# MMintLab/gelslim_depth

Hardware: AMD Instinct MI355X
Metric: train frames/sec (320x427) at batch 32 (higher is better)
Workload: dtype f32

## Files before the change

### gelslim_depth_amd/csrc/gsd_convT_wgrad.hip

```cpp
#include "gsd_wgrad_host.h"

template <int WM, int WN>
__global__ __launch_bounds__(256) void convT_wgrad_kernel(const WgradParams P) {
  constexpr int MT = 4, NTB = 4;
  constexpr int BMw = WM * 64, BNw = WN * 64;
  constexpr int DS = 66;

  extern __shared__ __attribute__((aligned(16))) float smem[];
  float* Al = smem;
  float* Xl = smem + BMw * DS;

  const int tid = threadIdx.x, lane = tid & 63, wave = tid >> 6;
  const int wm = wave / WN, wn = wave % WN;
  const int j = lane >> 4, l16 = lane & 15;

  const int per_split = P.mblocks * P.nblocks;
  const int split = blockIdx.x / per_split;
  const int rem = blockIdx.x - split * per_split;
  const int mb = rem % P.mblocks, nb = rem / P.mblocks;
  const int m0 = mb * BMw, n0 = nb * BNw;
  const int s_begin = (int)((long long)split * P.stages_total / P.splits);
  const int s_end = (int)((long long)(split + 1) * P.stages_total / P.splits);
  const int HW = P.H * P.W;

  f32x4 acc[MT][NTB];
#pragma unroll
  for (int m = 0; m < MT; ++m)
#pragma unroll
    for (int t = 0; t < NTB; ++t) acc[m][t] = f32x4{0.f, 0.f, 0.f, 0.f};

  const int q = tid & 63;
  const int lrow = tid >> 6;

  for (int stage = s_begin; stage < s_end; ++stage) {
    const int n = stage / P.tiles_flat;
    const int p = (stage - n * P.tiles_flat) * 64 + q;
    const bool pix_ok = p < HW;
    const int h = pix_ok ? p / P.W : 0;
    const int w = pix_ok ? p - h * P.W : 0;
    __syncthreads();
#pragma unroll
    for (int i = 0; i < BMw / 8; ++i) {
      const int rr = lrow + 4 * i;
      const int co = (m0 >> 2) + (rr >> 1);
      const int kh = rr & 1;
      float2 v = make_float2(0.f, 0.f);
      if (pix_ok && co < P.dy.C)
        v = *reinterpret_cast<const float2*>(P.dy.p + (long long)n * P.dy.ns + (long long)co * P.dy.cs +
                                             (long long)(2 * h + kh) * P.dy.W + 2 * w);
      const int mrow = (rr >> 1) * 4 + kh * 2;
      Al[mrow * DS + q] = v.x;
      Al[(mrow + 1) * DS + q] = v.y;
    }
#pragma unroll
    for (int i = 0; i < BNw / 4; ++i) {
      const int ch = lrow + 4 * i;
      const int c = n0 + ch;
      float v = 0.f;
      if (pix_ok && c < P.a0.C) {
        v = P.a0.p[(long long)n * P.a0.ns + (long long)c * P.a0.cs + p];
        if (P.a0.scale != nullptr) v = apply_affine(v, P.a0.scale[c], P.a0.shift[c], P.a0.relu);
        else if (P.a0.relu) v = fmaxf(v, 0.f);
      }
      Xl[ch * DS + q] = v;
    }
    __syncthreads();
    const int a_base = (wm * 64 + l16) * DS + j;
    const int b_base = (wn * 64 + l16) * DS + j;
    for (int s = 0; s < 16; ++s) {
      float a[MT], b[NTB];
#pragma unroll
      for (int m = 0; m < MT; ++m) a[m] = Al[a_base + m * 16 * DS + 4 * s];
#pragma unroll
      for (int t = 0; t < NTB; ++t) b[t] = Xl[b_base + t * 16 * DS + 4 * s];
#pragma unroll
      for (int m = 0; m < MT; ++m)
#pragma unroll
        for (int t = 0; t < NTB; ++t) acc[m][t] = mfma16(a[m], b[t], acc[m][t]);
    }
  }

#pragma unroll
  for (int m = 0; m < MT; ++m)
#pragma unroll
    for (int reg = 0; reg < 4; ++reg) {
      const int mr = m0 + wm * 64 + m * 16 + j * 4 + reg;
      if (mr < P.M) {
#pragma unroll
        for (int t = 0; t < NTB; ++t) {
          const int col = n0 + wn * 64 + t * 16 + l16;
          if (col < P.Ncols) P.slabs[((size_t)split * P.M + mr) * P.Ncols + col] = acc[m][t][reg];
        }
      }
    }
}

__device__ __attribute__((aligned(16))) const float gsd_zero16_wg[4] = {0.f, 0.f, 0.f, 0.f};
typedef float f32x2 __attribute__((ext_vector_type(2)));
template <int XM>
__global__ __launch_bounds__(256, 2) void convT_wgrad_dma_kernel(const WgradParams P) {
  constexpr bool BX = XM >= 1, AX = XM == 2;
  constexpr int MT = 4, NTB = 4, BMw = 128, BNw = 128, DS = 66, DSB = BX ? 64 : DS;
  extern __shared__ __attribute__((aligned(16))) float smem[];
  float* Al = smem;
  float* Bl = smem + BMw * DS;
  const int tid = threadIdx.x, lane = tid & 63;
  const int wave = __builtin_amdgcn_readfirstlane(tid >> 6);
  const int wm = wave >> 1, wn = wave & 1;
  const int j = lane >> 4, l16 = lane & 15;

  const int lid = xcd_swizzle(blockIdx.x, gridDim.x);
  const int per_split = P.mblocks * P.nblocks;
  const int split = lid / per_split;
  const int rem = lid - split * per_split;
  const int mb = rem % P.mblocks, nb = rem / P.mblocks;
  const int m0 = mb * BMw, n0 = nb * BNw;
  const int s_begin = (int)((long long)split * P.stages_total / P.splits);
  const int s_end = (int)((long long)(split + 1) * P.stages_total / P.splits);
  const int HW = P.H * P.W;

  float sc[NTB], sh[NTB], lo[NTB];
#pragma unroll
  for (int t = 0; t < NTB; ++t) {
    const int c = n0 + wn * 64 + t * 16 + l16;
    sc[t] = 1.f; sh[t] = 0.f; lo[t] = -__builtin_inff();
    if (c < P.a0.C) {
      if (P.a0.scale != nullptr) { sc[t] = P.a0.scale[c]; sh[t] = P.a0.shift[c]; }
      if (P.a0.relu) lo[t] = 0.f;
    }
  }

  f32x4 acc[MT][NTB];
#pragma unroll
  for (int m = 0; m < MT; ++m)
#pragma unroll
    for (int t = 0; t < NTB; ++t) acc[m][t] = f32x4{0.f, 0.f, 0.f, 0.f};

  const int a_off = AX ? (wm * 32 + (l16 >> 1)) * 128 + 2 * (j & 1) + (l16 & 1) : (wm * 64 + l16) * DS + j;
  const int a_lr = lane >> 5, a_q = lane & 31;
  const int a_sp = a_q ^ ((2 * wave + a_lr) & 7);
  const int b_off = (wn * 64 + l16) * DSB + j;
  const int b_lr = lane >> 4;
  const int b_piece = (lane & 15) ^ ((4 * wave + b_lr) & 15);
  for (int stage = s_begin; stage < s_end; ++stage) {
    const int n = stage / P.tiles_flat;
    const int p = (stage - n * P.tiles_flat) * 64 + lane;
    const bool pix_ok = p < HW;
    const int h = pix_ok ? p / P.W : 0;
    const int w = pix_ok ? p - h * P.W : 0;
    __syncthreads();
    f32x2 a_fix[AX ? BMw / 16 : 1];
    bool a_str = false;
    if constexpr (AX) {
      const int pa = (stage - n * P.tiles_flat) * 64 + 2 * a_sp;
      const bool pa_ok = pa < HW;
      const int ha = pa_ok ? pa / P.W : 0, wa = pa_ok ? pa - ha * P.W : 0;
      a_str = pa_ok && wa == P.W - 1;
      const bool pb_ok = pa + 1 < HW;
      const float* abase = P.dy.p + (long long)n * P.dy.ns + (long long)(2 * ha) * P.dy.W + 2 * wa;
#pragma unroll
      for (int i = 0; i < BMw / 16; ++i) {
        const int R = 2 * (wave + 4 * i) + a_lr;
        const int m = m0 + 2 * R;
        const float* src = abase + (long long)(m >> 2) * P.dy.cs + ((m >> 1) & 1) * P.dy.W;
        const float* gsrc = (pa_ok && m < P.M) ? src : &gsd_zero16_wg[0];
        float* dstp = Al + (wave + 4 * i) * 256;
        __builtin_amdgcn_global_load_lds(gsrc, dstp, 16, 0, 0);
        a_fix[i] = f32x2{0.f, 0.f};
        if (a_str && pb_ok && m < P.M) a_fix[i] = *reinterpret_cast<const f32x2*>(src + 2 * P.dy.W - 2 * wa);
      }
    } else {
      const float* abase = P.dy.p + (long long)n * P.dy.ns + (long long)(2 * h) * P.dy.W + 2 * w;
#pragma unroll 4
      for (int i = 0; i < BMw / 4; ++i) {
        const int row = wave + 4 * i;
        const int m = m0 + row;
        const float* gsrc = (pix_ok && m < P.M) ? abase + (long long)(m >> 2) * P.dy.cs + ((m >> 1) & 1) * P.dy.W + (m & 1) : &gsd_zero16_wg[0];
        __builtin_amdgcn_global_load_lds(gsrc, Al + row * DS, 4, 0, 0);
      }
    }
    if constexpr (BX) {
      const int p0 = (stage - n * P.tiles_flat) * 64 + 4 * b_piece;
      const bool pc_ok = p0 < HW;
      const float* bbase = P.a0.p + (long long)n * P.a0.ns + p0;
#pragma unroll 4
      for (int i = 0; i < BNw / 16; ++i) {
        const int ch = 4 * (wave + 4 * i) + b_lr;
        const int c = n0 + ch;
        const float* gsrc = (pc_ok && c < P.a0.C) ? bbase + (long long)c * P.a0.cs : &gsd_zero16_wg[0];
        float* dstp = Bl + (wave + 4 * i) * (4 * DSB);
        __builtin_amdgcn_global_load_lds(gsrc, dstp, 16, 0, 0);
      }
    } else {
      const float* bbase = P.a0.p + (long long)n * P.a0.ns + p;
#pragma unroll 4
      for (int i = 0; i < BNw / 4; ++i) {
        const int ch = wave + 4 * i;
        const int c = n0 + ch;
        const float* gsrc = (pix_ok && c < P.a0.C) ? bbase + (long long)c * P.a0.cs : &gsd_zero16_wg[0];
        __builtin_amdgcn_global_load_lds(gsrc, Bl + ch * DS, 4, 0, 0);
      }
    }
    if constexpr (AX) {
      __builtin_amdgcn_s_waitcnt(0x0F70);
      if (a_str) {
#pragma unroll
        for (int i = 0; i < BMw / 16; ++i)
          *reinterpret_cast<f32x2*>(&Al[(wave + 4 * i) * 256 + lane * 4 + 2]) = a_fix[i];
      }
      __syncthreads();
    } else {
      gsd_dma_barrier();
    }
    float an[MT], bn[NTB];
#pragma unroll
    for (int m = 0; m < MT; ++m) an[m] = AX ? Al[a_off + m * 8 * 128 + 4 * ((j >> 1) ^ (l16 >> 1))] : Al[a_off + m * 16 * DS];
#pragma unroll
    for (int t = 0; t < NTB; ++t) bn[t] = Bl[b_off + t * 16 * DSB + (BX ? 4 * l16 : 0)];
    for (int s = 0; s < 16; ++s) {
      float a[MT], b[NTB];
#pragma unroll
      for (int m = 0; m < MT; ++m) a[m] = an[m];
#pragma unroll
      for (int t = 0; t < NTB; ++t) b[t] = fmaxf(fmaf(bn[t], sc[t], sh[t]), lo[t]);
      const int sn = s + 1 < 16 ? s + 1 : s;
#pragma unroll
      for (int m = 0; m < MT; ++m)
        an[m] = AX ? Al[a_off + m * 8 * 128 + 4 * ((2 * sn + (j >> 1)) ^ (l16 >> 1))] : Al[a_off + m * 16 * DS + 4 * sn];
#pragma unroll
      for (int t = 0; t < NTB; ++t) bn[t] = Bl[b_off + t * 16 * DSB + 4 * (BX ? (sn ^ l16) : sn)];
#pragma unroll
      for (int m = 0; m < MT; ++m)
#pragma unroll
        for (int t = 0; t < NTB; ++t) acc[m][t] = mfma16(a[m], b[t], acc[m][t]);
    }
  }
#pragma unroll
  for (int m = 0; m < MT; ++m)
#pragma unroll
    for (int reg = 0; reg < 4; ++reg) {
      const int mr = m0 + wm * 64 + m * 16 + j * 4 + reg;
      if (mr < P.M) {
#pragma unroll
        for (int t = 0; t < NTB; ++t) {
          const int col = n0 + wn * 64 + t * 16 + l16;
          if (col < P.Ncols) P.slabs[((size_t)split * P.M + mr) * P.Ncols + col] = acc[m][t][reg];
        }
      }
    }
}

template <int LANES>
__global__ __launch_bounds__(LANES == 1 ? 256 : 64 * LANES) void convT_wgrad_reduce_kernel(const float* __restrict__ slabs,
                                                                                           float* __restrict__ dw, int splits, int M,
                                                                                           int Ncols) {
  constexpr int EL = LANES == 1 ? 256 : 64;
  const long long per = (long long)M * Ncols;
  const int el = threadIdx.x % EL, sl = threadIdx.x / EL;
  __shared__ float red[LANES][EL];
  for (long long e0 = (long long)blockIdx.x * EL; e0 < per; e0 += (long long)gridDim.x * EL) {
    const long long e = e0 + el;
    const bool ok = e < per;
    float s = 0.f;
    if (ok)
      for (int k = sl; k < splits; k += LANES) s += slabs[(size_t)k * per + e];
    if (LANES > 1) {
      red[sl][el] = s;
      __syncthreads();
      if (sl == 0) {
        s = 0.f;
#pragma unroll
        for (int i = 0; i < LANES; ++i) s += red[i][el];
      }
    }
    if (sl == 0 && ok) dw[(size_t)(e % Ncols) * M + (size_t)(e / Ncols)] = s;
    if (LANES > 1) __syncthreads();
  }
}

__global__ void sum_planes_stage1(const float* __restrict__ x, int N, int K, long long HW, float* __restrict__ ws) {
  const int k = blockIdx.x, g = blockIdx.y, G = gridDim.y;
  const long long total = (long long)N * HW;
  const long long per = (total + G - 1) / G;
  const long long b = (long long)g * per, e = b + per < total ? b + per : total;
  double s = 0.0;
  long long i = b + threadIdx.x;
  long long n = i / HW, p = i - n * HW;
  const long long step = blockDim.x, nstep = step / HW, pstep = step - nstep * HW;
  for (; i < e; i += step) {
    s += (double)x[((size_t)n * K + k) * HW + p];
    n += nstep;
    p += pstep;
    if (p >= HW) {
      p -= HW;
      ++n;
    }
  }
  __shared__ double red[16];
  s = wave_sum_d(s);
  if ((threadIdx.x & 63) == 0) red[threadIdx.x >> 6] = s;
  __syncthreads();
  if (threadIdx.x == 0) {
    double t = 0.0;
    for (int i = 0; i < (int)(blockDim.x >> 6); ++i) t += red[i];
    ws[(size_t)k * G + g] = (float)t;
  }
}
__global__ void sum_planes_stage2(const float* __restrict__ ws, int K, int G, float* __restrict__ out) {
  const int k = blockIdx.x * blockDim.x + threadIdx.x;
  if (k < K) {
    double s = 0.0;
    for (int g = 0; g < G; ++g) s += (double)ws[(size_t)k * G + g];
    out[k] = (float)s;
  }
}

namespace {

struct ConvTWgPlan {
  bool wide;
  int mblocks, nblocks, tiles_flat, stages_total, splits;
  int64_t slab_elems;
};

ConvTWgPlan plan_convT_wgrad(int N, int H, int W, int M, int Ncols) {
  ConvTWgPlan p;
  p.wide = M <= 64;
  p.mblocks = ceil_div(M, p.wide ? 64 : 128);
  p.nblocks = ceil_div(Ncols, p.wide ? 256 : 128);
  p.tiles_flat = ceil_div(H * W, 64);
  p.stages_total = N * p.tiles_flat;
  p.splits = wgrad_pick_splits(gsd_env_int("GSD_WGRAD_BLOCKS", 512), p.mblocks * p.nblocks, p.stages_total);
  p.slab_elems = (int64_t)p.splits * M * Ncols;
  return p;
}

void launch_convT_wgrad_reduce(const float* slabs, float* dw, int splits, int M, int Ncols, hipStream_t st) {
  const int lanes = splits >= 64 ? 16 : splits >= 8 ? 4 : 1;
  const int64_t blocks = ceil_div64((int64_t)M * Ncols, lanes == 1 ? 256 : 64), cap = lanes == 1 ? 4096 : 8192;
  const dim3 grid((int)(blocks < cap ? blocks : cap)), block(lanes == 1 ? 256 : 64 * lanes);
  if (lanes == 16) hipLaunchKernelGGL(convT_wgrad_reduce_kernel<16>, grid, block, 0, st, slabs, dw, splits, M, Ncols);
  else if (lanes == 4) hipLaunchKernelGGL(convT_wgrad_reduce_kernel<4>, grid, block, 0, st, slabs, dw, splits, M, Ncols);
  else hipLaunchKernelGGL(convT_wgrad_reduce_kernel<1>, grid, block, 0, st, slabs, dw, splits, M, Ncols);
}

}

extern "C" int64_t gsd_convT2x2_wgrad_workspace(int N, int H, int W, int Cin, int Cout) {
  if (N <= 0 || H <= 0 || W <= 0 || Cin <= 0 || Cout <= 0) return 0;
  return plan_convT_wgrad(N, H, W, Cout * 4, Cin).slab_elems + (int64_t)Cout * 64;
}

extern "C" int gsd_convT2x2_wgrad(const gsd_src* x, const gsd_src* dy, int Cin, int Cout, float* dw, float* dbias,
                                  float* workspace, int64_t workspace_elems, int N, int H, int W, void* stream) {
  GSD_REQUIRE(x && dy && dw && workspace, GSD_ERR_BAD_ARG, "gsd_convT2x2_wgrad: null argument");
  GSD_REQUIRE(N > 0 && H > 0 && W > 0 && Cin > 0 && Cout > 0, GSD_ERR_BAD_ARG, "gsd_convT2x2_wgrad: bad sizes");
  GSD_REQUIRE(x->ptr != nullptr && x->C == Cin && x->H == H && x->W == W && x->off_h == 0 && x->off_w == 0,
              GSD_ERR_BAD_ARG, "gsd_convT2x2_wgrad: x must be the full (Cin,H,W) tensor");
  GSD_REQUIRE((x->scale == nullptr) == (x->shift == nullptr), GSD_ERR_BAD_ARG,
              "gsd_convT2x2_wgrad: scale/shift must come together");
  if (int e = wgrad_check_plain(*dy, "gsd_convT2x2_wgrad dy")) return e;
  if (int e = gsd_require_rows_contiguous(*dy, "gsd_convT2x2_wgrad dy")) return e;
  if (int e = gsd_require_rows_contiguous(*x, "gsd_convT2x2_wgrad x")) return e;
  GSD_REQUIRE(dy->C == Cout && dy->H == 2 * H && dy->W == 2 * W, GSD_ERR_BAD_ARG,
              "gsd_convT2x2_wgrad: dy must be (Cout,2H,2W)");
  GSD_REQUIRE(((uintptr_t)dy->ptr & 7) == 0 && (dy->c_stride & 1) == 0 && (dy->n_stride & 1) == 0, GSD_ERR_UNSUPPORTED,
              "gsd_convT2x2_wgrad: dy must be 8-byte aligned with even strides");
  const int M = Cout * 4;
  const ConvTWgPlan pl = plan_convT_wgrad(N, H, W, M, Cin);
  const int64_t need = pl.slab_elems + (int64_t)Cout * 64;
  GSD_REQUIRE(workspace_elems >= need, GSD_ERR_WORKSPACE, "gsd_convT2x2_wgrad: workspace %lld < %lld elements",
              (long long)workspace_elems, (long long)need);
  WgradParams P{};
  wgrad_fill_common(P, x, 1, dy, Cin, M, workspace, N, H, W, pl.splits, pl.mblocks, pl.nblocks);
  P.Cact = Cin;
  P.tiles_flat = pl.tiles_flat;
  P.stages_total = pl.stages_total;
  const int grid = pl.splits * pl.mblocks * pl.nblocks;
  const size_t lds = (size_t)((pl.wide ? 64 + 256 : 128 + 128) * 66) * sizeof(float);
  const bool aligned = (H * W) % 4 == 0 && ((uintptr_t)x->ptr & 15) == 0 && x->c_stride % 4 == 0 && x->n_stride % 4 == 0;
  const char* const what = "gsd_convT2x2_wgrad";
  const hipStream_t st = (hipStream_t)stream;
  if (int e = pl.wide   ? gsd_launch<convT_wgrad_kernel<1, 4>>(what, dim3(grid), dim3(256), lds, st, P)
              : aligned ? gsd_launch<convT_wgrad_dma_kernel<2>>(what, dim3(grid), dim3(256), lds, st, P)
                        : gsd_launch<convT_wgrad_dma_kernel<0>>(what, dim3(grid), dim3(256), lds, st, P))
    return e;
  launch_convT_wgrad_reduce(workspace, dw, pl.splits, M, Cin, st);
  GSD_LAUNCH_CHECK("gsd_convT2x2_wgrad reduce");
  if (dbias != nullptr) {
    GSD_REQUIRE(dy->c_stride == (int64_t)4 * H * W && dy->n_stride == (int64_t)Cout * 4 * H * W, GSD_ERR_UNSUPPORTED,
                "gsd_convT2x2_wgrad: bias gradient needs a contiguous dy");
    float* ws2 = workspace + pl.slab_elems;
    hipLaunchKernelGGL(sum_planes_stage1, dim3(Cout, 64), dim3(256), 0, (hipStream_t)stream, dy->ptr, N, Cout,
                       (long long)4 * H * W, ws2);
    GSD_LAUNCH_CHECK("gsd_convT2x2_wgrad bias stage1");
    hipLaunchKernelGGL(sum_planes_stage2, dim3(ceil_div(Cout, 256)), dim3(256), 0, (hipStream_t)stream, ws2, Cout, 64,
                       dbias);
    GSD_LAUNCH_CHECK("gsd_convT2x2_wgrad bias stage2");
  }
  return GSD_OK;
}

extern "C" int gsd_sum_planes(const float* x, int N, int K, int64_t HW, float* out, float* workspace, void* stream) {
  GSD_REQUIRE(x && out && workspace && N > 0 && K > 0 && HW > 0, GSD_ERR_BAD_ARG, "gsd_sum_planes: bad argument");
  hipLaunchKernelGGL(sum_planes_stage1, dim3(K, 64), dim3(K <= 8 ? 1024 : 256), 0, (hipStream_t)stream, x, N, K, (long long)HW, workspace);
  GSD_LAUNCH_CHECK("gsd_sum_planes stage1");
  hipLaunchKernelGGL(sum_planes_stage2, dim3(ceil_div(K, 256)), dim3(256), 0, (hipStream_t)stream, workspace, K, 64, out);
  GSD_LAUNCH_CHECK("gsd_sum_planes stage2");
  return GSD_OK;
}
```

### gelslim_depth_amd/engine.py

```python
from __future__ import annotations

import ctypes as C
import os
from typing import Dict, List, Optional, Sequence

import torch

from . import _lib as L
from ._lib import lib, check
from .engine_base import BN_EPS, ConvUnit, EngineBase, UpUnit


def _r64(c: int) -> int:
    return (c + 63) // 64 * 64


def _r4(w: int) -> int:
    return (w + 3) // 4 * 4


class _ConvForm:

    def __init__(self, algo: int):
        self.algo = algo
        self.conv = (lib.gsd_conv3x3, lib.gsd_conv3x3_w43, lib.gsd_conv3x3_w2d)[algo]
        self.dgrad_bnrelu = (lib.gsd_conv3x3_dgrad_bnrelu, lib.gsd_conv3x3_w43_dgrad_bnrelu, lib.gsd_conv3x3_w2d_dgrad_bnrelu)[algo]
        self.partial_rows = (lib.gsd_conv3x3_partial_rows, lib.gsd_conv3x3_w43_partial_rows, lib.gsd_conv3x3_w2d_partial_rows)[algo]
        self.mode_f, self.mode_d = ((0, 1), (4, 5), (8, 9))[algo]
        self.workspace = (lambda *a: 0, lib.gsd_conv3x3_w43_workspace, lib.gsd_conv3x3_w2d_workspace)[algo]

    @staticmethod
    def choose(n: int, h: int, w: int, cin: int, c0: int, cout: int, train: bool) -> "_ConvForm":
        if not train:
            algo = lib.gsd_conv3x3_algo(1, h, w, cin, cout)
            if algo == 1:
                algo = 2 if lib.gsd_conv3x3_w2d_supported(cin, c0) else 0
            return _ConvForm(algo)
        algo = lib.gsd_conv3x3_algo(n, h, w, cin, cout)
        if algo == 1 and lib.gsd_conv3x3_w2d_supported(cin, c0) and lib.gsd_conv3x3_prefers_w2d(n, h, w, cin, cout, int(train)):
            algo = 2
        return _ConvForm(algo)

    def run(self, ws, src, nsrc, wt, cin, cout, dst, ndst, part, n, h, w, st):
        if self.algo >= 1 and ws is not None:
            fn = lib.gsd_conv3x3_w43_ws if self.algo == 1 else lib.gsd_conv3x3_w2d_ws
            return fn(src, nsrc, wt, cin, cout, dst, ndst, part, ws.data_ptr(), ws.numel(), n, h, w, st)
        return self.conv(src, nsrc, wt, cin, cout, dst, ndst, part, n, h, w, st)

    def run_bnrelu(self, ws, src, wt, cin, cout, dst, raw, scale, shift, mean, invstd, part, n, h, w, st):
        if self.algo >= 1 and ws is not None:
            fn = lib.gsd_conv3x3_w43_dgrad_bnrelu_ws if self.algo == 1 else lib.gsd_conv3x3_w2d_dgrad_bnrelu_ws
            return fn(src, wt, cin, cout, dst, raw, scale, shift, mean, invstd, part, ws.data_ptr(), ws.numel(), n, h, w, st)
        return self.dgrad_bnrelu(src, wt, cin, cout, dst, raw, scale, shift, mean, invstd, part, n, h, w, st)


class _Unit(ConvUnit):
    def __init__(self, prefix: str, conv_idx: int, bn_idx: int, cin: int, cout: int, level: int):
        super().__init__(prefix, conv_idx, bn_idx, cin, cout, level)
        self.c0 = cin
        self.raw = None
        self.dsrc = None
        self.pitched = False
        self.fused_dw = False
        self.srcs = None
        self.act_once = False
        self.form_f = self.form_d = None
        self.forms_f = None


class _Up(UpUnit):
    def __init__(self, j: int, cin: int, level_in: int):
        super().__init__(j, cin, level_in)
        self.mode_d = 3
        self.bn_rows = 0
        self.out = self.dout = None
        self.cat = None


class UNetEngine(EngineBase):
    Unit, Up = _Unit, _Up

    def __init__(self, n_channels: int, n_classes: int, layer_dimensions: Sequence[int]):
        super().__init__(n_channels, n_classes, layer_dimensions)
        for j, (u0, _) in enumerate(self.dec):
            u0.c0 = self.dims[self.L - 1 - j]
        self._saved = False
        self._saved_eval = False
        self.one_launch_rows = int(os.environ.get("GSD_BN_ONE_LAUNCH_ROWS", "4096"))
        self.side_dw = os.environ.get("GSD_SIDE_DW", "1") != "0"
        self.wgrad_log: Optional[list] = None

    _SIZING_ENV = ("GSD_W2D_TW", "GSD_W2D_TW8_PCT", "GSD_W43_TW", "GSD_W43_FOLD", "GSD_CONV_W2D", "GSD_CONV_ALGO", "GSD_W43_SPLIT",
                   "GSD_WGRAD_ALGO", "GSD_WGRAD_W2D", "GSD_WG2D_KX", "GSD_WG2D_BLOCKS", "GSD_WGRAD_BLOCKS", "GSD_WG43_TW",
                   "GSD_ACT_ONCE", "GSD_ACT_ONCE_FORCE", "GSD_W2D_X4")

    @staticmethod
    def _desc(c: int, h: int, w: int, pitch: int, deferred: bool = False, n: int = 1) -> L.gsd_src:
        s = L.gsd_src()
        s.ptr = 256
        s.scale = s.shift = 256 if deferred else None
        s.C, s.H, s.W, s.relu, s.w_stride, s.slack = c, h, w, int(deferred), pitch, L.SLACK
        s.c_stride = h * pitch
        s.n_stride = c * h * pitch
        return s

    def _dw_form(self, u: "_Unit", n: int, lh: int, lw: int, segs) -> int:
        arr = L.src_array(segs)
        pitched = bool(lib.gsd_conv3x3_wgrad_takes_pitched_dy(n, lh, lw, u.cin, u.cout)) and (not u.need_dgrad or u.form_d.algo >= 1)
        dy = self._desc(u.cout, lh, lw, _r4(lw) if pitched else lw)
        return lib.gsd_conv3x3_wgrad_form(arr, len(segs), C.byref(dy), u.cin, u.cout, n, lh, lw)

    def _plan_act_once(self, n: int) -> None:
        on = os.environ.get("GSD_ACT_ONCE", "1") != "0"
        hs, ws = self.hs, self.ws
        self.pooled_pitched = [False] * (self.L + 1)
        self.cat_on = [False] * self.L
        for u in self.units:
            u.act_once = False
        if not on:
            return
        w2d = lambda u: all(f.algo == 2 for f in u.forms_f.values())
        for lvl, (u0, u1) in enumerate(self.enc):
            lh, lw = hs[lvl], ws[lvl]
            if lvl >= 1 and w2d(u0) and lib.gsd_act_once_pays(n, lh, lw, u0.cin, u0.cin, u0.cout, 0, 0, 2) and \
                    lib.gsd_conv3x3_wgrad_takes_pitched_act(n, lh, lw, u0.cin, u0.cout) and \
                    self._dw_form(u0, n, lh, lw, [self._desc(u0.cin, lh, lw, lw)]) == \
                    self._dw_form(u0, n, lh, lw, [self._desc(u0.cin, lh, lw, _r4(lw))]):
                self.pooled_pitched[lvl] = True
        for pair in self.enc + self.dec:
            u0, u1 = pair
            lh, lw = hs[u1.level], ws[u1.level]
            u1.act_once = u1.forms_f[True].algo == 2 and bool(lib.gsd_act_once_pays(n, lh, lw, u1.cin, u1.cin, u1.cout, 0, 0, 0))
        for j, (u0, _) in enumerate(self.dec):
            lvl = self.L - 1 - j
            lh, lw = hs[lvl], ws[lvl]
            cs, cu = u0.c0, u0.cin - u0.c0
            p = _r4(lw)
            two = [self._desc(cs, lh, lw, lw, deferred=True), self._desc(cu, 2 * hs[lvl + 1], 2 * ws[lvl + 1], 2 * ws[lvl + 1])]
            self.cat_on[j] = self._pad_off(lvl) == (0, 0) and w2d(u0) and \
                bool(lib.gsd_act_once_pays(n, lh, lw, cs, u0.cin, u0.cout, 0, 0, 1)) and \
                bool(lib.gsd_conv3x3_wgrad_takes_pitched_act(n, lh, lw, u0.cin, u0.cout)) and \
                self._dw_form(u0, n, lh, lw, two) == self._dw_form(u0, n, lh, lw, [self._desc(u0.cin, lh, lw, p)])

    def _ensure(self, n: int, h: int, w: int, dev: torch.device, train: bool) -> None:
        key = (n, h, w, str(dev), self._env_key())
        if self._shape == key and (not train or self.units[0].g is not None):
            return
        if self._shape != key:
            for u in self.units:
                u.raw = u.g = None
            for up in self.ups:
                up.out = up.dout = up.cat = None
        self._shape = key
        hs, ws = self._set_pyramid(h, w)
        f32 = dict(device=dev, dtype=torch.float32)
        max_part = 1
        max_ws = 1
        max_gp = 0
        max_slab = 0
        for u in self.units:
            lh, lw = hs[u.level], ws[u.level]
            if u.raw is None:
                u.raw = L.slack_empty((n, u.cout, lh, lw), dev)
            if train and u.g is None:
                u.g = torch.empty((n, u.cout, lh, lw), **f32)
            self._alloc_bn(u, dev)
            u.forms_f = {t: _ConvForm.choose(n, lh, lw, u.cin, u.c0, u.cout, t) for t in (False, True)}
            u.form_f = u.forms_f[train]
            u.form_d = _ConvForm.choose(n, lh, lw, u.cout, u.cout, u.cin, True) if u.need_dgrad else None
            need = max(lib.gsd_weight_layout_size(f.mode_f, u.cout, u.cin) for f in u.forms_f.values())
            if u.wt_f is None or u.wt_f.numel() != need or u.wt_f.device != dev:
                u.wt_f = torch.empty((need,), **f32)
            if not u.need_dgrad and train:
                need = lib.gsd_weight_layout_size(1, u.cout, u.cin)
                if u.wt_d is None or u.wt_d.numel() != need or u.wt_d.device != dev:
                    u.wt_d = torch.empty((need,), **f32)
            if u.need_dgrad:
                need = lib.gsd_weight_layout_size(u.form_d.mode_d, u.cout, u.cin)
                if u.wt_d is None or u.wt_d.numel() != need or u.wt_d.device != dev:
                    u.wt_d = torch.empty((need,), **f32)
                max_part = max(max_part, u.form_d.partial_rows(n, lh, lw, u.cin) * 2 * _r64(u.cin))
            rows = max(f.partial_rows(n, lh, lw, u.cout) for f in u.forms_f.values())
            max_part = max(max_part, rows * 2 * _r64(u.cout))
            if train:
                max_slab = max(max_slab, u.form_f.workspace(n, lh, lw, u.cin, u.cout),
                               u.form_d.workspace(n, lh, lw, u.cout, u.cin) if u.need_dgrad else 0)
                max_part = max(max_part, lib.gsd_bn_bwd_partial_rows(n, u.cout, lh, lw) * 3 * u.cout)
                max_ws = max(max_ws, lib.gsd_conv3x3_wgrad_workspace(n, lh, lw, u.cin, u.cout))
                u.pitched = bool(lib.gsd_conv3x3_wgrad_takes_pitched_dy(n, lh, lw, u.cin, u.cout)) and \
                    (not u.need_dgrad or u.form_d.algo >= 1)
                if u.pitched:
                    max_gp = max(max_gp, n * u.cout * lh * _r4(lw))
                u.fused_dw = (not u.need_dgrad) and bool(lib.gsd_conv3x3_wgrad_bn_supported(n, lh, lw, u.cin, u.cout))
                if u.fused_dw:
                    max_ws = max(max_ws, lib.gsd_conv3x3_wgrad_bn_workspace(n, lh, lw, u.cin, u.cout))
        self._plan_act_once(n)
        max_act = max([n * u.cin * hs[u.level] * _r4(ws[u.level]) for u in self.units if u.act_once] + [0])
        self.act_buf = torch.empty((max_act,), **f32) if (train and max_act) else None
        for up in self.ups:
            li = up.level_in
            if up.out is None and self.cat_on[up.j]:
                up.cat = L.pitched_slack_zeros((n, 2 * up.cout, hs[li - 1], ws[li - 1]), dev)
                up.out = up.cat[:, up.cout:, :2 * hs[li], :2 * ws[li]]
            if up.out is None:
                up.out = L.slack_empty((n, up.cout, 2 * hs[li], 2 * ws[li]), dev)
            if train and up.dout is None:
                up.dout = L.slack_empty((n, up.cout, 2 * hs[li], 2 * ws[li]), dev)
            if up.wt_f is None or up.wt_f.device != dev:
                up.wt_f = torch.empty((lib.gsd_weight_layout_size(6, up.cout, up.cin),), **f32)
            if train:
                up.mode_d = lib.gsd_convT2x2_dgrad_layout(C.byref(L.make_src(up.dout, slack=L.SLACK)), up.cin, up.cout, n, hs[li], ws[li])
                need = lib.gsd_weight_layout_size(up.mode_d, up.cout, up.cin)
                if up.wt_d is None or up.wt_d.numel() != need or up.wt_d.device != dev:
                    up.wt_d = torch.empty((need,), **f32)
                up.bn_rows = 0
                if up.mode_d == 7:
                    up.bn_rows = lib.gsd_convT2x2_dgrad_bnrelu_partial_rows(C.byref(L.make_src(up.dout, slack=L.SLACK)), up.cin,
                                                                            up.cout, n, hs[li], ws[li])
                    max_part = max(max_part, up.bn_rows * 2 * _r64(up.cin))
            if train:
                max_ws = max(max_ws, lib.gsd_convT2x2_wgrad_workspace(n, hs[li], ws[li], up.cin, up.cout))
        self.pooled = [None] + [(L.pitched_slack_zeros if self.pooled_pitched[l] else L.slack_empty)((n, self.dims[l - 1], hs[l], ws[l]), dev)
                                for l in range(1, self.L + 1)]
        self.dpooled = [None] + ([torch.empty((n, self.dims[l - 1], hs[l], ws[l]), **f32)
                                 for l in range(1, self.L + 1)] if train else [None] * self.L)
        side = train and self.side_dw
        self.side = torch.cuda.Stream(device=dev) if side else None
        self.gps = [torch.empty((max_gp,), **f32) for _ in range(2 if side else 1)] if (train and max_gp) else None
        self.gp_turn = 0
        self.gp_free: List[Optional[torch.cuda.Event]] = [None, None]
        self.partials = torch.empty((max_part,), **f32)
        self.conv_ws = torch.empty((max_slab,), **f32) if (train and max_slab) else None
        self.db_sums = torch.empty((65 * 2 * max(u.cin for u in self.units),), device=dev, dtype=torch.float64) if train else None
        self.wgrad_ws = torch.empty((max(max_ws, 64 * max(1, self.n_classes)),), **f32) if train else None
        self.wgrad_ws_side = torch.empty((max(max_ws, 64),), **f32) if side else None
        self.outw_partials = self.outw_sums = None
        if train and self.n_classes > 1:
            kc = self.n_classes * self.dims[0]
            self.outw_partials = torch.empty((lib.gsd_conv1x1_out_wgrad_rows(n, hs[0], ws[0]) * kc,), **f32)
            self.outw_sums = torch.empty((65 * kc,), device=dev, dtype=torch.float64)

    @staticmethod
    def _layouts(jobs, st: int) -> None:
        arr = (L.gsd_wl_job * len(jobs))()
        for i, (mode, w, co, ci, wt) in enumerate(jobs):
            arr[i].w, arr[i].wt, arr[i].mode, arr[i].Co, arr[i].Ci = w.data_ptr(), wt.data_ptr(), mode, co, ci
        check(lib.gsd_weight_layout_batch(arr, len(jobs), st), "weight_layout_batch")

    @staticmethod
    def _act_src(u: _Unit) -> L.gsd_src:
        return L.make_src(u.raw, u.scale, u.shift, relu=True, slack=L.SLACK)

    def _activate(self, prev: _Unit, dst_t: torch.Tensor, st: int) -> None:
        s, d = self._act_src(prev), L.make_dst(dst_t)
        check(lib.gsd_bnrelu_pitched(C.byref(s), C.byref(d), prev.raw.shape[0], st), "bnrelu_pitched")

    def _run_unit(self, u: _Unit, srcs: List[L.gsd_src], P: Dict[str, torch.Tensor], train: bool, st: int,
                  keep: bool = False, prev: Optional[_Unit] = None) -> None:
        n = u.raw.shape[0]
        lh, lw = self.hs[u.level], self.ws[u.level]
        u.form_f = u.forms_f[train]
        u.srcs = L.src_array(srcs)
        arr = u.srcs
        if train and prev is not None and u.act_once:
            p = _r4(lw)
            act = self.act_buf[:n * u.cin * lh * p].view(n, u.cin, lh, p)[..., :lw]
            self._activate(prev, act, st)
            srcs = [L.make_src(act)]
            arr = L.src_array(srcs)
        dst = L.dst_array([L.make_dst(u.raw)])
        part = self.partials.data_ptr() if train else None
        ev = self._log_begin()
        check(u.form_f.run(self.conv_ws if train else None, arr, len(srcs), u.wt_f.data_ptr(), u.cin, u.cout, dst, 1, part,
                           n, lh, lw, st), "conv3x3")
        self._log_end(ev, u.cout, u.cin, n, lh, lw, u.form_f.algo)
        if train:
            rows = u.form_f.partial_rows(n, lh, lw, u.cout)
            self._bn_stats(u, rows, _r64(u.cout), float(n * lh * lw), P, st,
                           one_launch=self.sync_fn is None and rows <= self.one_launch_rows)
        elif keep:
            check(lib.gsd_bn_eval_coeffs_bwd(P[u.gname].data_ptr(), P[u.bname].data_ptr(), P[u.rmname].data_ptr(),
                                             P[u.rvname].data_ptr(), BN_EPS, u.cout, u.scale.data_ptr(), u.shift.data_ptr(),
                                             u.mean.data_ptr(), u.invstd.data_ptr(), st),
                  "bn_eval_coeffs_bwd")
        else:
            check(lib.gsd_bn_eval_coeffs(P[u.gname].data_ptr(), P[u.bname].data_ptr(), P[u.rmname].data_ptr(),
                                         P[u.rvname].data_ptr(), BN_EPS, u.cout, u.scale.data_ptr(), u.shift.data_ptr(), st),
                  "bn_eval_coeffs")

    def _log_begin(self):
        if self.kernel_log is None and self.region_log is None:
            return None
        return self._event()

    def _log_end(self, ev, m: int, k_ch: int, n: int, lh: int, lw: int, algo: int = 0) -> None:
        if ev is None or self.kernel_log is None:
            return
        e = self._event()
        flops = 2.0 * m * k_ch * 9 * n * lh * lw
        if algo == 2:
            variant = "conv3x3_w2d_kernel"
            executed = 2048.0 * lib.gsd_conv3x3_w2d_mfma_count(n, lh, lw, k_ch, m)
        elif algo:
            variant = "conv3x3_w43_kernel"
            executed = 2048.0 * lib.gsd_conv3x3_w43_mfma_count(n, lh, lw, k_ch, m)
        else:
            variant = "conv3x3_dma_kernel<1,4>" if m <= 64 else "conv3x3_dma_kernel<2,2>"
            executed = flops
        self.kernel_log.append((variant, flops, ev, e, (m, k_ch, lh, lw), executed))

    def forward(self, x: torch.Tensor, P: Dict[str, torch.Tensor], train: bool, out: Optional[torch.Tensor] = None,
                keep: bool = False) -> torch.Tensor:
        keep = keep and not train
        x = self._begin_forward(x, train or keep)
        n, _, h, w = x.shape
        st = L.stream_ptr()
        self._saved = train or keep
        self._saved_eval = keep
        self._layouts([(u.forms_f[train].mode_f, P[u.wname], u.cout, u.cin, u.wt_f) for u in self.units] +
                      [(6, P[up.wname], up.cout, up.cin, up.wt_f) for up in self.ups], st)
        region = self._log_begin() if self.region_log is not None else None
        for lvl in range(self.L + 1):
            u0, u1 = self.enc[lvl]
            if lvl == 0:
                srcs = [L.make_src(x)]
            else:
                if lvl == 1 and region is not None:
                    self.region_log.append(("inc_forward", region, self._event()))
                prev = self.enc[lvl - 1][1]
                s = self._act_src(prev)
                cat = self.ups[self.L - lvl].cat if train and self.cat_on[self.L - lvl] else None
                skip_t = None if cat is None else cat[:, :prev.cout]
                if self.pooled_pitched[lvl]:
                    dp = L.make_dst(self.pooled[lvl])
                    da = None if skip_t is None else C.byref(L.make_dst(skip_t))
                    check(lib.gsd_maxpool2_pitched(C.byref(s), C.byref(dp), da, n, st), "maxpool2_pitched")
                else:
                    check(lib.gsd_maxpool2(C.byref(s), self.pooled[lvl].data_ptr(), n, prev.cout, self.hs[lvl - 1],
                                           self.ws[lvl - 1], st), "maxpool2")
                    if skip_t is not None:
                        self._activate(prev, skip_t, st)
                srcs = [L.make_src(self.pooled[lvl], slack=L.SLACK)]
            self._run_unit(u0, srcs, P, train, st, keep)
            self._run_unit(u1, [self._act_src(u0)], P, train, st, keep, prev=u0)
        if self.L == 0 and region is not None:
            self.region_log.append(("inc_forward", region, self._event()))
        cur = self.enc[self.L][1]
        for j in range(self.L):
            up = self.ups[j]
            lvl = self.L - 1 - j
            s = self._act_src(cur)
            d = L.make_dst(up.out)
            check(lib.gsd_convT2x2(C.byref(s), up.wt_f.data_ptr(), P[up.bname].data_ptr(), up.cin, up.cout, C.byref(d), n,
                                   self.hs[lvl + 1], self.ws[lvl + 1], st), "convT2x2")
            skip = self.enc[lvl][1]
            u0, u1 = self.dec[j]
            if train and self.cat_on[j]:
                self._run_unit(u0, [L.make_src(up.cat, slack=L.SLACK)], P, train, st, keep)
            else:
                self._run_unit(u0, [self._act_src(skip), L.make_src(up.out, off=self._pad_off(lvl), slack=L.SLACK)], P, train, st,
                               keep)
            self._run_unit(u1, [self._act_src(u0)], P, train, st, keep, prev=u0)
            cur = u1
        self._flush_counters()
        if out is None:
            out = torch.empty((n, self.n_classes, h, w), device=x.device, dtype=torch.float32)
        s = self._act_src(cur)
        check(lib.gsd_conv1x1_out(C.byref(s), P["outc.conv.weight"].data_ptr(), P["outc.conv.bias"].data_ptr(), cur.cout,
                                  self.n_classes, out.data_ptr(), n, h, w, st), "conv1x1_out")
        return out

    def _bn_bwd_tail(self, u: _Unit, P, G, st: int, dwout: Optional[torch.Tensor] = None, fused: bool = False) -> None:
        n = u.raw.shape[0]
        lh, lw = self.hs[u.level], self.ws[u.level]
        rows = u.fused_rows if fused else lib.gsd_bn_bwd_partial_rows(n, u.cout, lh, lw)
        self._bn_bwd_sums(u, rows, _r64(u.cout) if fused else 0, float(n * lh * lw), G, dwout, st,
                          one_launch=self.sync_fn is None and rows <= self.one_launch_rows and (dwout is None or not fused))
        if self._saved_eval:
            u.c1.zero_()
            u.c2.zero_()
        if u.fused_dw:
            self._on_side(lambda sst, ws: check(
                lib.gsd_conv3x3_wgrad_bn(u.srcs, u.g.data_ptr(), u.raw.data_ptr(), u.scale.data_ptr(), u.mean.data_ptr(),
                                         u.invstd.data_ptr(), u.c1.data_ptr(), u.c2.data_ptr(), u.cin, u.cout,
                                         G[u.wname].data_ptr(), ws.data_ptr(), ws.numel(), n, lh, lw, sst), "conv3x3_wgrad_bn"))
            return
        turn = None
        if u.pitched:
            p = _r4(lw)
            turn = self.gp_turn = (self.gp_turn + 1) % len(self.gps)
            if self.gp_free[turn] is not None:
                torch.cuda.current_stream().wait_event(self.gp_free[turn])
                self.gp_free[turn] = None
            u.dsrc = self.gps[turn][:n * u.cout * lh * p].view(n, u.cout, lh, p)[..., :lw]
            out_ptr = u.dsrc.data_ptr()
        else:
            p, u.dsrc, out_ptr = 0, u.g, None
# ... 157 lines not shown
```

Baseline: 388.1.

## Add triple-buffered 256x128 pipelined kernel for transposed-conv weight gradient

Adds a new 512-thread ConvTranspose2x2 weight-gradient kernel that uses a 256x128 output tile with 32-pixel K stages. Global data is moved into LDS with direct-to-LDS DMA loads in a three-stage ring, and the fill/publish, the deferred BN+ReLU activation pass and the MFMA steps are interleaved under explicit scheduling barriers. Split-K is now sized to the CU count and blocks are XCD-swizzled. The kernel is taken when M is a multiple of 256, Cin a multiple of 128 and the data is aligned; otherwise the old kernels run. In exchange it uses more LDS, runs at one block per CU, and adds an odd-width fixup path that raises correctness risk.

After: 391.7 (median of 6 runs). Within noise of the previous version (+0.9%).

```diff
diff --git a/gelslim_depth_amd/csrc/gsd_convT_wgrad.hip b/gelslim_depth_amd/csrc/gsd_convT_wgrad.hip
--- a/gelslim_depth_amd/csrc/gsd_convT_wgrad.hip
+++ b/gelslim_depth_amd/csrc/gsd_convT_wgrad.hip
@@ -250,6 +250,250 @@
     }
 }
 
+template <bool PLAIN>
+__global__ __launch_bounds__(512, 1) void convT_wgrad_pipe_kernel(const WgradParams P) {
+  constexpr int AB = 128 * 64 * 4, XB = 128 * 32 * 4, IMG = AB + XB;
+  extern __shared__ __attribute__((aligned(16))) float smem[];
+  char* const lds = reinterpret_cast<char*>(smem);
+  const int tid = threadIdx.x, lane = tid & 63;
+  const int wave = __builtin_amdgcn_readfirstlane(tid >> 6);
+  const int wm = wave >> 1, wn = wave & 1;
+  const int j = lane >> 4, l16 = lane & 15;
+
+  const int lid = xcd_swizzle(blockIdx.x, gridDim.x);
+  const int per_split = P.mblocks * P.nblocks;
+  const int split = lid / per_split;
+  const int rem = lid - split * per_split;
+  const int mb = rem % P.mblocks, nb = rem / P.mblocks;
+  const int m0 = mb * 256, n0 = nb * 128;
+  const int s_begin = (int)((long long)split * P.stages_total / P.splits);
+  const int s_end = (int)((long long)(split + 1) * P.stages_total / P.splits);
+  const int nst = s_end - s_begin;
+  const int W = P.W, HW = P.H * P.W;
+  const int odd = W & 1;
+
+  int f_t, f_h0, f_w0;
+  const char *dy_img, *x_img;
+  {
+    const int n = s_begin / P.tiles_flat;
+    f_t = s_begin - n * P.tiles_flat;
+    f_h0 = (f_t * 32) / W;
+    f_w0 = f_t * 32 - f_h0 * W;
+    dy_img = reinterpret_cast<const char*>(P.dy.p + (long long)n * P.dy.ns + (long long)(m0 >> 2) * P.dy.cs);
+    x_img = reinterpret_cast<const char*>(P.a0.p + (long long)n * P.a0.ns + (long long)n0 * P.a0.cs);
+  }
+  const int dq = 32 / W, dr = 32 - dq * W;
+  const long long dy_cs4 = P.dy.cs * 4, x_cs4 = P.a0.cs * 4;
+
+  const int a_lr = lane >> 4;
+  const int a_sp = (lane & 15) ^ (4 * (wave & 3) + a_lr);
+  const int a_ph = (2 * a_sp) / W, a_pw = 2 * a_sp - a_ph * W;
+  const unsigned a_lane = (unsigned)((a_lr >> 1) * dy_cs4) + (unsigned)((a_lr & 1) * P.dy.W * 4) + (unsigned)((4 * a_sp + 2 * W * a_ph) * 4);
+  const int b_piece = (lane & 7) ^ (4 * (wave & 1) + (lane >> 4));
+  const unsigned b_lane = (unsigned)((lane >> 3) * x_cs4) + (unsigned)(b_piece * 16);
+
+  f32x2 sc[2], sh[2], lo2;
+  if constexpr (!PLAIN) {
+#pragma unroll
+    for (int i = 0; i < 2; ++i) {
+      const int c = n0 + (tid >> 3) + 64 * i;
+      const float s = P.a0.scale != nullptr ? P.a0.scale[c] : 1.f, t = P.a0.scale != nullptr ? P.a0.shift[c] : 0.f;
+      sc[i] = f32x2{s, s};
+      sh[i] = f32x2{t, t};
+      asm volatile("" : "+v"(sc[i]), "+v"(sh[i]));
+    }
+    const float lo = P.a0.relu ? 0.f : -__builtin_inff();
+    lo2 = f32x2{lo, lo};
+  }
+
+  unsigned a_rd[2][2], b_rd[2];
+#pragma unroll
+  for (int h = 0; h < 2; ++h) {
+#pragma unroll
+    for (int e = 0; e < 2; ++e) a_rd[h][e] = (unsigned)((wm * 32 + l16) * 256 + (((8 * h + 2 * j + e) ^ l16) * 16));
+    b_rd[h] = (unsigned)(AB + (wn * 64 + l16) * 128 + (((4 * h + j) ^ (l16 >> 1)) * 16));
+  }
+
+  f32x4 acc[2][2][4];
+#pragma unroll
+  for (int g = 0; g < 2; ++g)
+#pragma unroll
+    for (int k = 0; k < 2; ++k)
+#pragma unroll
+      for (int t = 0; t < 4; ++t) acc[g][k][t] = f32x4{0.f, 0.f, 0.f, 0.f};
+
+  f32x2 a_fix[4];
+  bool a_str = false;
+  auto dma = [&](const char* src, char* dst) __attribute__((always_inline)) {
+    __builtin_amdgcn_global_load_lds(reinterpret_cast<const float*>(src), reinterpret_cast<float*>(dst), 16, 0, 0);
+  };
+  auto fill = [&](const int buf) __attribute__((always_inline)) {
+    char* const img = lds + buf * IMG;
+    const int p0 = f_t * 32;
+    unsigned a_off = a_lane + (a_pw >= W - f_w0 ? (unsigned)(8 * W) : 0u);
+    asm volatile("" : "+v"(a_off));
+    const char* const dyb = dy_img + (long long)(2 * p0 + 2 * W * f_h0) * 4;
+    const char* const xb = x_img + (long long)p0 * 4;
+    unsigned bl = b_lane;
+    asm volatile("" : "+v"(bl));
+    auto a_src = [&](const int i) __attribute__((always_inline)) {
+      const char* b = dyb + (2 * wave + 16 * i) * dy_cs4;
+      asm volatile("" : "+s"(b));
+      return b;
+    };
+    auto b_src = [&](const int i) __attribute__((always_inline)) {
+      const char* b = xb + (8 * wave + 64 * i) * x_cs4;
+      asm volatile("" : "+s"(b));
+      return b;
+    };
+    bool str = odd != 0 && a_pw == W - 1 - f_w0;
+    if (p0 + 32 <= HW) {
+#pragma unroll
+      for (int i = 0; i < 4; ++i) dma(a_src(i) + a_off, img + (wave + 8 * i) * 1024);
+#pragma unroll
+      for (int i = 0; i < 2; ++i) dma(b_src(i) + bl, img + AB + (wave + 8 * i) * 1024);
+    } else {
+      const bool a_ok = p0 + 2 * a_sp < HW, b_ok = p0 + 4 * b_piece < HW;
+      const char* const zero = reinterpret_cast<const char*>(&gsd_zero16_wg[0]);
+      str = str && a_ok;
+#pragma unroll
+      for (int i = 0; i < 4; ++i) dma(a_ok ? a_src(i) + a_off : zero, img + (wave + 8 * i) * 1024);
+#pragma unroll
+      for (int i = 0; i < 2; ++i) dma(b_ok ? b_src(i) + bl : zero, img + AB + (wave + 8 * i) * 1024);
+    }
+    if (odd) {
+      if (str) {
+        const unsigned f_off = a_off + (unsigned)((2 * W + 2) * 4);
+#pragma unroll
+        for (int i = 0; i < 4; ++i) a_fix[i] = *reinterpret_cast<const f32x2*>(a_src(i) + f_off);
+      }
+    }
+    a_str = str;
+    ++f_t;
+    f_w0 += dr;
+    f_h0 += dq;
+    if (f_w0 >= W) {
+      f_w0 -= W;
+      ++f_h0;
+    }
+    if (f_t == P.tiles_flat) {
+      f_t = 0; f_h0 = 0; f_w0 = 0;
+      dy_img += P.dy.ns * 4;
+      x_img += P.a0.ns * 4;
+    }
+  };
+  auto publish = [&](const int buf) __attribute__((always_inline)) {
+    if (odd) {
+      __builtin_amdgcn_s_waitcnt(0x0F70);
+      if (a_str) {
+#pragma unroll
+        for (int i = 0; i < 4; ++i) *reinterpret_cast<f32x2*>(lds + buf * IMG + (wave + 8 * i) * 1024 + lane * 16 + 8) = a_fix[i];
+      }
+    }
+    a_str = false;
+    gsd_dma_barrier();
+  };
+  f32x4 raw[2];
+  auto act_rd = [&](const int buf) __attribute__((always_inline)) {
+#pragma unroll
+    for (int i = 0; i < 2; ++i) raw[i] = *reinterpret_cast<const f32x4*>(lds + buf * IMG + AB + (tid + 512 * i) * 16);
+  };
+  auto act_wr = [&](const int buf) __attribute__((always_inline)) {
+#pragma unroll
+    for (int i = 0; i < 2; ++i) {
+      const f32x2 v0 = __builtin_elementwise_max(__builtin_elementwise_fma(f32x2{raw[i][0], raw[i][1]}, sc[i], sh[i]), lo2);
+      const f32x2 v1 = __builtin_elementwise_max(__builtin_elementwise_fma(f32x2{raw[i][2], raw[i][3]}, sc[i], sh[i]), lo2);
+      *reinterpret_cast<f32x4*>(lds + buf * IMG + AB + (tid + 512 * i) * 16) = f32x4{v0[0], v0[1], v1[0], v1[1]};
+    }
+  };
+
+  f32x4 Ar[2][2][2], Br[2][4];
+  auto rd = [&](const int buf, const int h) __attribute__((always_inline)) {
+#pragma unroll
+    for (int t = 0; t < 4; ++t) Br[h][t] = *reinterpret_cast<const f32x4*>(lds + buf * IMG + t * 2048 + b_rd[h]);
+#pragma unroll
+    for (int g = 0; g < 2; ++g)
+#pragma unroll
+      for (int e = 0; e < 2; ++e) Ar[h][g][e] = *reinterpret_cast<const f32x4*>(lds + buf * IMG + g * 4096 + a_rd[h][e]);
+  };
+  auto mmk = [&](const int h, const int e, const int s) __attribute__((always_inline)) {
+#pragma unroll
+    for (int g = 0; g < 2; ++g)
+#pragma unroll
+      for (int k = 0; k < 2; ++k)
+#pragma unroll
+        for (int t = 0; t < 4; ++t) acc[g][k][t] = mfma16(Ar[h][g][e][2 * s + k], Br[h][t][2 * e + s], acc[g][k][t]);
+  };
+  auto mm = [&](const int h, const int e) __attribute__((always_inline)) {
+    mmk(h, e, 0);
+    mmk(h, e, 1);
+  };
+
+  fill(0);
+  publish(0);
+  if (nst > 1) {
+    fill(1);
+    publish(1);
+  }
+  if constexpr (!PLAIN) {
+    act_rd(0);
+    act_wr(0);
+    if (nst > 1) {
+      act_rd(1);
+      act_wr(1);
+    }
+  }
+  if (nst > 2) fill(2);
+  __syncthreads();
+  rd(0, 0);
+
+  auto step = [&](auto cur_c, const int it) __attribute__((always_inline)) {
+    constexpr int cur = decltype(cur_c)::value, nxt = (cur + 1) % 3, nn = (cur + 2) % 3;
+    mm(0, 0);
+    __builtin_amdgcn_sched_barrier(0);
+    rd(cur, 1);
+    __builtin_amdgcn_sched_barrier(0);
+    mm(0, 1);
+    __builtin_amdgcn_sched_barrier(0);
+    publish(nn);
+    __builtin_amdgcn_sched_barrier(0);
+    mmk(1, 0, 0);
+    __builtin_amdgcn_sched_barrier(0);
+    if (it + 3 < nst) fill(cur);
+    if constexpr (!PLAIN)
+      if (it + 2 < nst) act_rd(nn);
+    __builtin_amdgcn_sched_barrier(0);
+    mmk(1, 0, 1);
+    __builtin_amdgcn_sched_barrier(0);
+    if constexpr (!PLAIN)
+      if (it + 2 < nst) act_wr(nn);
+    if (it + 1 < nst) rd(nxt, 0);
+    __builtin_amdgcn_sched_barrier(0);
+    mm(1, 1);
+    __builtin_amdgcn_sched_barrier(0);
+  };
+  typedef std::integral_constant<int, 0> I0;
+  typedef std::integral_constant<int, 1> I1;
+  typedef std::integral_constant<int, 2> I2;
+  for (int it = 0; it < nst; it += 3) {
+    step(I0{}, it);
+    if (it + 1 < nst) step(I1{}, it + 1);
+    if (it + 2 < nst) step(I2{}, it + 2);
+  }
+
+  float* const out = P.slabs + ((size_t)split * P.M + m0) * P.Ncols + n0 + wn * 64 + l16;
+#pragma unroll
+  for (int g = 0; g < 2; ++g)
+#pragma unroll
+    for (int reg = 0; reg < 4; ++reg)
+#pragma unroll
+      for (int k = 0; k < 2; ++k) {
+        const int mr = 2 * (wm * 32 + g * 16 + j * 4 + reg) + k;
+#pragma unroll
+        for (int t = 0; t < 4; ++t) out[(size_t)mr * P.Ncols + t * 16] = acc[g][k][t][reg];
+      }
+}
+
 template <int LANES>
 __global__ __launch_bounds__(LANES == 1 ? 256 : 64 * LANES) void convT_wgrad_reduce_kernel(const float* __restrict__ slabs,
                                                                                            float* __restrict__ dw, int splits, int M,
@@ -335,6 +579,29 @@
   return p;
 }
 
+struct ConvTWgPipePlan {
+  bool ok;
+  int mblocks, nblocks, tiles_flat, stages_total, splits;
+  int64_t slab_elems;
+};
+
+ConvTWgPipePlan plan_convT_wgrad_pipe(int N, int H, int W, int M, int Ncols) {
+  ConvTWgPipePlan p{};
+  const int64_t hw = (int64_t)H * W;
+  p.ok = gsd_env_int("GSD_CONVT_WG_PIPE", 1) != 0 && M % 256 == 0 && Ncols % 128 == 0 && hw % 4 == 0 && hw < (1 << 26) &&
+         (int64_t)N * ceil_div64(hw, 32) < (1 << 30);
+  if (!p.ok) return p;
+  p.mblocks = M / 256;
+  p.nblocks = Ncols / 128;
+  p.tiles_flat = ceil_div(H * W, 32);
+  p.stages_total = N * p.tiles_flat;
+  const int forced = gsd_env_int("GSD_CONVT_WG_SPLITS", 0);
+  p.splits = forced > 0 ? (forced < p.stages_total ? forced : p.stages_total)
+                        : wgrad_pick_splits(gsd_cu_count(), p.mblocks * p.nblocks, p.stages_total);
+  p.slab_elems = (int64_t)p.splits * M * Ncols;
+  return p;
+}
+
 void launch_convT_wgrad_reduce(const float* slabs, float* dw, int splits, int M, int Ncols, hipStream_t st) {
   const int lanes = splits >= 64 ? 16 : splits >= 8 ? 4 : 1;
   const int64_t blocks = ceil_div64((int64_t)M * Ncols, lanes == 1 ? 256 : 64), cap = lanes == 1 ? 4096 : 8192;
@@ -348,7 +615,8 @@
 
 extern "C" int64_t gsd_convT2x2_wgrad_workspace(int N, int H, int W, int Cin, int Cout) {
   if (N <= 0 || H <= 0 || W <= 0 || Cin <= 0 || Cout <= 0) return 0;
-  return plan_convT_wgrad(N, H, W, Cout * 4, Cin).slab_elems + (int64_t)Cout * 64;
+  const int64_t a = plan_convT_wgrad(N, H, W, Cout * 4, Cin).slab_elems, b = plan_convT_wgrad_pipe(N, H, W, Cout * 4, Cin).slab_elems;
+  return (a > b ? a : b) + (int64_t)Cout * 64;
 }
 
 extern "C" int gsd_convT2x2_wgrad(const gsd_src* x, const gsd_src* dy, int Cin, int Cout, float* dw, float* dbias,
@@ -367,7 +635,14 @@
   GSD_REQUIRE(((uintptr_t)dy->ptr & 7) == 0 && (dy->c_stride & 1) == 0 && (dy->n_stride & 1) == 0, GSD_ERR_UNSUPPORTED,
               "gsd_convT2x2_wgrad: dy must be 8-byte aligned with even strides");
   const int M = Cout * 4;
-  const ConvTWgPlan pl = plan_convT_wgrad(N, H, W, M, Cin);
+  const bool aligned = (H * W) % 4 == 0 && ((uintptr_t)x->ptr & 15) == 0 && x->c_stride % 4 == 0 && x->n_stride % 4 == 0;
+  ConvTWgPlan pl = plan_convT_wgrad(N, H, W, M, Cin);
+  const ConvTWgPipePlan pp = plan_convT_wgrad_pipe(N, H, W, M, Cin);
+  const bool pipe = pp.ok && aligned && x->c_stride < (1 << 25) && dy->c_stride < (1 << 26);
+  if (pipe) {
+    pl.mblocks = pp.mblocks; pl.nblocks = pp.nblocks; pl.tiles_flat = pp.tiles_flat; pl.stages_total = pp.stages_total;
+    pl.splits = pp.splits; pl.slab_elems = pp.slab_elems;
+  }
   const int64_t need = pl.slab_elems + (int64_t)Cout * 64;
   GSD_REQUIRE(workspace_elems >= need, GSD_ERR_WORKSPACE, "gsd_convT2x2_wgrad: workspace %lld < %lld elements",
               (long long)workspace_elems, (long long)need);
@@ -378,10 +653,14 @@
   P.stages_total = pl.stages_total;
   const int grid = pl.splits * pl.mblocks * pl.nblocks;
   const size_t lds = (size_t)((pl.wide ? 64 + 256 : 128 + 128) * 66) * sizeof(float);
-  const bool aligned = (H * W) % 4 == 0 && ((uintptr_t)x->ptr & 15) == 0 && x->c_stride % 4 == 0 && x->n_stride % 4 == 0;
   const char* const what = "gsd_convT2x2_wgrad";
   const hipStream_t st = (hipStream_t)stream;
-  if (int e = pl.wide   ? gsd_launch<convT_wgrad_kernel<1, 4>>(what, dim3(grid), dim3(256), lds, st, P)
+  if (pipe) {
+    const size_t lds3 = (size_t)3 * (128 * 64 + 128 * 32) * sizeof(float);
+    if (int e = (x->scale == nullptr && x->relu == 0) ? gsd_launch<convT_wgrad_pipe_kernel<true>>(what, dim3(grid), dim3(512), lds3, st, P)
+                                                      : gsd_launch<convT_wgrad_pipe_kernel<false>>(what, dim3(grid), dim3(512), lds3, st, P))
+      return e;
+  } else if (int e = pl.wide   ? gsd_launch<convT_wgrad_kernel<1, 4>>(what, dim3(grid), dim3(256), lds, st, P)
               : aligned ? gsd_launch<convT_wgrad_dma_kernel<2>>(what, dim3(grid), dim3(256), lds, st, P)
                         : gsd_launch<convT_wgrad_dma_kernel<0>>(what, dim3(grid), dim3(256), lds, st, P))
     return e;
diff --git a/gelslim_depth_amd/engine.py b/gelslim_depth_amd/engine.py
--- a/gelslim_depth_amd/engine.py
+++ b/gelslim_depth_amd/engine.py
@@ -92,7 +92,7 @@
 
     _SIZING_ENV = ("GSD_W2D_TW", "GSD_W2D_TW8_PCT", "GSD_W43_TW", "GSD_W43_FOLD", "GSD_CONV_W2D", "GSD_CONV_ALGO", "GSD_W43_SPLIT",
                    "GSD_WGRAD_ALGO", "GSD_WGRAD_W2D", "GSD_WG2D_KX", "GSD_WG2D_BLOCKS", "GSD_WGRAD_BLOCKS", "GSD_WG43_TW",
-                   "GSD_ACT_ONCE", "GSD_ACT_ONCE_FORCE", "GSD_W2D_X4")
+                   "GSD_ACT_ONCE", "GSD_ACT_ONCE_FORCE", "GSD_W2D_X4", "GSD_CONVT_WG_PIPE", "GSD_CONVT_WG_SPLITS")
 
     @staticmethod
     def _desc(c: int, h: int, w: int, pitch: int, deferred: bool = False, n: int = 1) -> L.gsd_src:
```
